# ViennaRNA/RNAcode

Measured on AMD Instinct MI355X. Metric: alignment-columns x samples scored /sec, higher is better.
Workload: dtype f32; 1 GPU; synthetic MAF 10000 blocks x 120 cols x 6 seqs, n=1000 (BASELINE configs[2]/[3]); exchange=none, fit_exp_mode=fused

## Files before the change

rnacode_amd/csrc/rc_batch.cpp:

```cpp
#include "rc_runtime.h"


extern "C" {

void rc_batch_destroy(rc_batch *b) {
  if (!b) return;
  trace("destroy", b);
  (void)hipSetDevice(b->device);
  const bool ctxAlive = b->ctx && !(b->retiredKeep && b->retiredKeep->ctxGone.load());
  if (b->state == rc_batch::RUNNING) { if (b->evDone.e) (void)hipEventSynchronize(b->evDone); if (ctxAlive) b->ctx->inflight.fetch_sub(1); }
  else if (b->state == rc_batch::READY && b->evPrep.e) (void)hipEventSynchronize(b->evPrep);
  delete b;
  trace("destroyed", b);
}

}


extern "C" void rc_batch_destroy(rc_batch *b);

int batch_prepare(rc_batch *b, const rc_block *blocks, int32_t n_blocks, const rc_params *par, const TableSet *set) {
  rc_ctx *ctx = b->ctx;
  if (par->blosum != 62 && par->blosum != 90) return fail(RC_ERR_ARG, "blosum must be 62 or 90");
  if (par->sampleN < 1) return fail(RC_ERR_ARG, "sampleN must be >= 1");
// ... 15 lines not shown
    if (blocks[i].n_rows >= 3 && blocks[i].n_rows <= kMaxRows && blocks[i].n_cols >= 3 && blocks[i].n_cols <= RC_MAX_COLS)
      block_footprint(blocks[i].n_rows, blocks[i].n_cols, &h, &d);
    hostSum += h; devSum += d;
  }
  const size_t nn = static_cast<size_t>(std::max(n_blocks, 1));
  const size_t tail = al256(nn * sizeof(DevBlock)) + 2 * al256(nn * sizeof(int)) + al256(nn * sizeof(uint64_t)) + al256((nn + 1) * sizeof(int));
  b->hostCap = al256(hostSum) + tail + 256;
  b->devCap = al256(devSum) + 256;
  HIP_TRY(hipSetDevice(ctx->device));
  HIP_TRY(b->hblob.ensure(b->hostCap));
  BlobArena arena;
  arena.host = b->hblob.as<uint8_t>();
  arena.hostCap = b->hostCap;
  arena.devCap = b->devCap;

  {
    if (!ctx->pool || ctx->pool->size() != ctx->hostThreads) ctx->pool.reset(new Pool(ctx->hostThreads));
    std::mutex errMu;
    ctx->pool->run(n_blocks, [&](int i) {
      std::string err;
      const int st = prepare_block(blocks[i], *par, pt, arena, static_cast<uint32_t>(i), b->db[i], b->meta[i], err);
      if (st != RC_OK && st != RC_ERR_SKIP) {
        std::lock_guard<std::mutex> lk(errMu);
        b->errs[i] = err;
      }
    });
  }

  bool sameL = true;
  const size_t SpadBytes = (static_cast<size_t>(par->sampleN) + kWave - 1) / kWave * kWave * sizeof(uint32_t);
  for (int i = 0; i < n_blocks; i++) {
    BlockMeta &m = b->meta[i];
    if (m.status != RC_OK) continue;
    if (static_cast<double>(b->db[i].nnodes) * m.cols * static_cast<double>(SpadBytes) > static_cast<double>(ctx->totalMem) / 4.0) {
      m.status = RC_ERR_UNSUPPORTED; b->db[i].status = RC_ERR_UNSUPPORTED;
      b->errs[i] = "rows x columns x samples too large for the device: the block's random-number streams (4 bytes x tree nodes x columns x samples) exceed a quarter of its memory; split the block (breakmaf) or lower --num-samples";
      continue;
    }
    b->okBlocks.push_back(i);
    auto &cls = b->classes[block_class(m.N, m.L, b->db[i].omega, ctx->rule)];
    if (!cls.empty() && b->meta[cls.front()].L != m.L) sameL = false;
    cls.push_back(i);
    b->maxL = std::max(b->maxL, m.L);
    b->maxDraws = std::max(b->maxDraws, b->db[i].nnodes * m.cols);
    const size_t smax = static_cast<size_t>(m.L) / 3;
    b->hssCap = std::max(b->hssCap, static_cast<int>(smax) / 3 + 2);
  }
  if (!sameL)
    for (auto &kv : b->classes) std::stable_sort(kv.second.begin(), kv.second.end(), [&](int x, int y) { return b->meta[x].L > b->meta[y].L; });
  for (auto &kv : b->classes)
    if (kv.first > kGenericClass) std::stable_sort(kv.second.begin(), kv.second.end(), [&](int x, int y) { return b->meta[x].NK > b->meta[y].NK; });

  uint8_t *base = arena.host;
  size_t o = al256(arena.hostUsed.load());
  auto take = [&](size_t bytes) { const size_t at = o; o += al256(bytes); return at; };
  b->oDblocks = take(nn * sizeof(DevBlock));
  b->oOk = take(nn * sizeof(int));
  b->oClass = take(nn * sizeof(int));
  b->oPrefix = take((nn + 1) * sizeof(int));
  if (o > b->hostCap) return fail(RC_ERR_ARG, "internal: blob tail does not fit");
  b->hostUsed = o;
  if (n_blocks > 0) std::memcpy(base + b->oDblocks, b->db.data(), sizeof(DevBlock) * n_blocks);
  if (!b->okBlocks.empty()) std::memcpy(base + b->oOk, b->okBlocks.data(), sizeof(int) * b->okBlocks.size());
  {
    int *cl = reinterpret_cast<int *>(base + b->oClass);
    int at = 0;
    std::fill(b->classOff, b->classOff + kClassSlots, 0);
// ... 337 lines not shown
```

rnacode_amd/csrc/rc_host.cpp:

```cpp
#include "rc_host.h"
#include "rc_refexp.h"

#include <algorithm>
#include <cmath>
#include <cstdlib>
#include <cstring>
#include <vector>

namespace rc {

static inline float f32(double x) { return static_cast<float>(x); }
static inline double f64(float x) { return static_cast<double>(x); }


namespace {
bool fast_decimal(const char *p, const char **end, double *out) {
  static const double pow10[23] = {1e0, 1e1, 1e2, 1e3, 1e4, 1e5, 1e6, 1e7, 1e8, 1e9, 1e10, 1e11, 1e12, 1e13, 1e14, 1e15, 1e16, 1e17, 1e18, 1e19, 1e20, 1e21, 1e22};
  const char *q = p;
  bool neg = false;
  if (*q == '-' || *q == '+') { neg = (*q == '-'); q++; }
  unsigned long long m = 0;
  int digits = 0, frac = 0, any = 0;
  for (; *q >= '0' && *q <= '9'; q++) { any = 1; if (m || *q != '0') { m = m * 10 + static_cast<unsigned>(*q - '0'); digits++; } if (digits > 15) return false; }
  if (*q == '.') {
    q++;
    for (; *q >= '0' && *q <= '9'; q++) { any = 1; m = m * 10 + static_cast<unsigned>(*q - '0'); if (m) digits++; frac++; if (digits > 15 || frac > 22) return false; }
  }
  if (!any || *q == 'e' || *q == 'E' || *q == 'x' || *q == 'X' || *q == 'p' || *q == 'P') return false;
  const double v = static_cast<double>(m) / pow10[frac];
  *out = neg ? -v : v;
  *end = q;
  return true;
}
// ... 410 lines not shown
    uint8_t *dst = chars + static_cast<size_t>(r) * cols;
    const uint8_t *src = reinterpret_cast<const uint8_t *>(in.rows[r]);
    for (int c = 0; c < cols; c++) dst[c] = luts.up[src[c]];
  }

  tip_distances(t, rowtip, N, dist, mark);
  float freqs[2][4];
  mono_freqs_both(chars, static_cast<size_t>(N) * cols, freqs[0], freqs[1]);
  ModelRec *models = reinterpret_cast<ModelRec *>(base + d.off_models);
  for (int s = 0; s < 2; s++)
    for (int j = 0; j < N; j++) {
      ModelRec &m = models[s * N + j];
      std::memset(&m, 0, sizeof m);
      m.dist = dist[j];
      m.kappa = in.kappa;
      std::memcpy(m.freqs, freqs[s], sizeof m.freqs);
      hky_probs(m.dist, m.freqs, m.kappa, m.P);
    }

  SeqGenHky hky(freqs[0], in.kappa);
  NodeRec *nodes = reinterpret_cast<NodeRec *>(base + d.off_nodes);
  for (int q = 0; q < t.nnodes; q++) {
    NodeRec &nr = nodes[q];
    std::memset(&nr, 0, sizeof nr);
    nr.parent = static_cast<uint16_t>(t.parent[q]);
    nr.gctrl = node_ctrl(static_cast<uint32_t>(t.parent[q])) | ((t.parent[q] >> 3) == (q >> 3) ? 0x80000000u : 0u);
    nr.tiprow = -1;
    double M[4][4];
    if (q != 0) hky.cumulative(t.length[q], M);
    for (int p = 0; p < 4; p++) {
      uint32_t b = 0;
      pack_thresholds(q == 0 ? hky.addFreq : M[p], &nr.thr[p], &b);
      nr.basepack |= b << (2 * p);
    }
  }
  uint8_t *qtip = base + d.off_qtip;
  uint16_t *qtip16 = reinterpret_cast<uint16_t *>(base + d.off_qtip16);
  std::memset(qtip, 0, sec.qtip);
  for (int r = 0; r < N; r++) {
    const int q = t.tipnode[rowtip[r]];
    qtip[r] = static_cast<uint8_t>(q);
    qtip16[r] = static_cast<uint16_t>(q);
    nodes[q].tiprow = static_cast<int16_t>(r);
  }
  return done(RC_OK);
}

int exp_mode_of_host() {
  bool fused = true, generic = true;
  uint64_t s = 88172645463325252ull;
  for (int i = 0; i < 20000 && (fused || generic); i++) {
    s ^= s << 13; s ^= s >> 7; s ^= s << 17;
    const double u = static_cast<double>(s >> 11) * (1.0 / 9007199254740992.0);
    const double x = (i & 3) == 3 ? 709.7 * u : -745.2 * u;
    const uint64_t want = exp_bits(std::exp(x));
    if (fused && exp_bits(ref_exp(x, true)) != want) fused = false;
    if (generic && exp_bits(ref_exp(x, false)) != want) generic = false;
  }
  return fused ? 2 : generic ? 1 : 0;
}

float pvalue_of(float score, float parMu, float parLambda) {
  const float arg = (-1) * parLambda * (score - parMu);
  return f32(1 - std::exp((-1) * std::exp(f64(arg))));
}

// ... 8 lines not shown
```

rnacode_amd/csrc/rc_null_generic.h:

```cpp
#pragma once
#include "rc_null_kernel.h"
#include "rc_null_tiled.h"

namespace rc {

struct GenericLayout {
  size_t offCodes;
  size_t offState;
  size_t offRow;
  size_t total;
  int nW;
  __host__ __device__ GenericLayout(int N, int L, int nn) {
    const size_t NK = static_cast<size_t>(N) - 1;
    nW = ((L / 3 + 31) >> 2) + 1;
    offCodes = 0;
    offState = (offCodes + 6 * NK * static_cast<size_t>(nW) * kWave * sizeof(uint32_t) + 255) & ~static_cast<size_t>(255);
    (void)nn;
    offRow = (offState + 2 * (3 * NK + 1) * kWave * sizeof(float) + 255) & ~static_cast<size_t>(255);
    total = (offRow + (static_cast<size_t>(L) / 3 + 8) * kWave * sizeof(float) + 255) & ~static_cast<size_t>(255);
  }
};

__host__ __device__ inline size_t generic_codes_bytes(int N, int L, int nn) { return GenericLayout(N, L, nn).offState; }
__host__ __device__ inline size_t generic_state_bytes(int N, int L, int nn) { const GenericLayout l(N, L, nn); return l.total - l.offState; }
// ... 157 lines not shown
#pragma unroll
          for (int t = 0; t < 8; t++) { u[t] = *up; up += qstride; }
        } else {
#pragma unroll
          for (int t = 0; t < 8; t++) {
            u[t] = 0u;
            if (q0 + t < nnodes) { u[t] = *up; up += qstride; }
          }
        }
        const int qa = q0 + thrNode < lastNode ? q0 + thrNode : lastNode, qb = q0 + 4 + thrNode < lastNode ? q0 + 4 + thrNode : lastNode;
        ta = nodew[qa * 20 + thrLane];
        tb = nodew[qb * 20 + thrLane];
        const int qc = q0 + (lane & 7) < lastNode ? q0 + (lane & 7) : lastNode;
        cv = nodew[qc * 20 + 16 + ((lane >> 3) & 3)];
      };
      fetch(0, uu, thrA, thrB, ctlV);
      for (int q0 = 0; q0 < nnodes; q0 += 8) {
        uint32_t un[8], tnA = 0u, tnB = 0u, cnV = 0u;
        if (q0 + 8 < nnodes) fetch(q0 + 8, un, tnA, tnB, cnV);
        const bool full = q0 + 8 <= nnodes;
        uint32_t cur = 0u;
        auto node = [&](auto tc) {
          constexpr int t = decltype(tc)::value;
          const uint32_t bp = static_cast<uint32_t>(__builtin_amdgcn_readlane(static_cast<int>(ctlV), t));
          const uint32_t ctl = static_cast<uint32_t>(__builtin_amdgcn_readlane(static_cast<int>(ctlV), 16 + t));
          uint32_t pw = cur;
          if (static_cast<int>(ctl) >= 0) pw = *reinterpret_cast<const uint16_t *>(ldsBytes + ((ctl & 0x7f80u) | laneSt));
          const uint32_t ps = (pw >> (ctl & 31u)) & 3u;
          const int at = static_cast<int>(ps << 4) + (t & 3) * 64;
          const int tv = static_cast<int>(t < 4 ? thrA : thrB);
          const uint32_t thx = static_cast<uint32_t>(__builtin_amdgcn_ds_bpermute(at, tv)), thy = static_cast<uint32_t>(__builtin_amdgcn_ds_bpermute(at + 4, tv)),
                         thz = static_cast<uint32_t>(__builtin_amdgcn_ds_bpermute(at + 8, tv)), thw = static_cast<uint32_t>(__builtin_amdgcn_ds_bpermute(at + 12, tv));
          const uint32_t u = uu[t];
          const uint32_t st = (u > thx) + (u > thy) + (u > thz) + ((bp >> (2 * ps)) & 3u);
          clamped += (u > thw);
          cur |= (st & 3u) << (2 * t);
        };
        if (full) {
          static_for<8>(node);
        } else {
          static_for<8>([&](auto tc) { if (q0 + decltype(tc)::value < nnodes) node(tc); });
        }
        *reinterpret_cast<uint16_t *>(ldsBytes + (static_cast<uint32_t>(q0 >> 3) * 128u + laneSt)) = static_cast<uint16_t>(cur);
#pragma unroll
        for (int t = 0; t < 8; t++) uu[t] = un[t];
        thrA = tnA; thrB = tnB; ctlV = cnV;
      }
      const int ip = L + 3 - i;
      const int jF = i / 3 - 1, jR = ip / 3 - 1;
      const uint32_t offF = (static_cast<uint32_t>(0 + i % 3) * NK * lay.nW + static_cast<uint32_t>(jF >> 2)) * (kWave * 4) + lane * 4 + (jF & 3);
      const uint32_t offR = (static_cast<uint32_t>(3 + ip % 3) * NK * lay.nW + static_cast<uint32_t>(jR >> 2)) * (kWave * 4) + lane * 4 + (jR & 3);
      const uint32_t *__restrict__ mrowF = maskw + static_cast<size_t>(0 * L1 + i) * NCW, *__restrict__ mrowR = maskw + static_cast<size_t>(1 * L1 + (i >= 3 ? ip : L)) * NCW;
      const bool emit = i >= 3;
      uint32_t aF, aR;
      {
        const uint32_t c = node_ctrl(qtip[0]);
        const uint32_t wv = *reinterpret_cast<const uint16_t *>(ldsBytes + ((c & 0x7f80u) | laneSt));
        aF = ((static_cast<uint32_t>(win[0]) << 2) | ((wv >> (c & 31u)) & 3u)) & 63u;
        win[0] = static_cast<uint8_t>(aF);
        aR = codon_flip(aF) ^ 63u;
      }
      const uint32_t aF64 = aF * 64u, aR64 = aR * 64u;
      uint8_t *__restrict__ kp = codes;
      const size_t kstep = static_cast<size_t>(lay.nW) * (kWave * 4);
      const int kChunk = TILED ? (kWave / A.tiledKT) * A.tiledKT : kWave;
      for (int k0 = 0; k0 < NK; k0 += kChunk) {
        const int kl = k0 + lane < NK ? k0 + lane : NK - 1;
        const uint32_t tctl = node_ctrl(qtip[kl + 1]);
        const uint32_t k5 = static_cast<uint32_t>(kl) / 5u, sh = 6u * (static_cast<uint32_t>(kl) - 5u * k5);
        const uint32_t mFv = (mrowF[k5] >> sh) & 63u, mRv = (mrowR[k5] >> sh) & 63u;
        const int nk = NK - k0 < kWave ? NK - k0 : kWave;
        if constexpr (TILED) {
          const TiledLayout tl(NK, A.tiledKT);
          uint32_t *__restrict__ cwp = reinterpret_cast<uint32_t *>(codes) + lane;
          const size_t posF = static_cast<size_t>(0 * L1 + i) * tl.WT * kWave, posR = static_cast<size_t>(1 * L1 + (emit ? ip : L)) * tl.WT * kWave;
          auto rowsT = [&](auto cnt, int kk, int widx) {
            constexpr int CNT = decltype(cnt)::value;
            uint32_t bb[CNT], cc[CNT], wv[CNT];
            uint8_t *wrow = win + (kk + 1) * kWave;
#pragma unroll
            for (int t = 0; t < CNT; t++) {
              cc[t] = static_cast<uint32_t>(__builtin_amdgcn_readlane(static_cast<int>(tctl), kk - k0 + t));
              wv[t] = *reinterpret_cast<const uint16_t *>(ldsBytes + ((cc[t] & 0x7f80u) | laneSt));
              bb[t] = wrow[t * kWave];
            }
#pragma unroll
            for (int t = 0; t < CNT; t++) bb[t] = ((bb[t] << 2) | ((wv[t] >> (cc[t] & 31u)) & 3u)) & 63u;
#pragma unroll
            for (int t = 0; t < CNT; t++) wrow[t * kWave] = static_cast<uint8_t>(bb[t]);
            if (emit) {
              uint32_t wf = 0u, wr = 0u;
#pragma unroll
              for (int t = 0; t < CNT; t++) {
                const uint32_t mF = static_cast<uint32_t>(__builtin_amdgcn_readlane(static_cast<int>(mFv), kk - k0 + t));
                const uint32_t mR = static_cast<uint32_t>(__builtin_amdgcn_readlane(static_cast<int>(mRv), kk - k0 + t));
                wf |= static_cast<uint32_t>(pairTab[aF64 + (bb[t] & mF)]) << (6 * t + 2);
                wr |= static_cast<uint32_t>(pairTab[aR64 + ((codon_flip(bb[t]) ^ 63u) & mR)]) << (6 * t + 2);
              }
              cwp[posF + static_cast<size_t>(widx) * kWave] = wf;
              cwp[posR + static_cast<size_t>(widx) * kWave] = wr;
            }
          };
          const int t0 = k0 / tl.KT, t1 = t0 + kChunk / tl.KT < tl.T ? t0 + kChunk / tl.KT : tl.T;
          for (int t = t0; t < t1; t++)
            for (int x = 0; x < tl.WPT; x++) {
              const int kk = t * tl.KT + 5 * x;
              int cnt = tl.KT - 5 * x;
              cnt = cnt > 5 ? 5 : cnt;
              cnt = cnt > NK - kk ? NK - kk : cnt;
              const int widx = t * tl.WPT + x;
              if (cnt >= 5) rowsT(std::integral_constant<int, 5>{}, kk, widx);
              else if (cnt == 4) rowsT(std::integral_constant<int, 4>{}, kk, widx);
              else if (cnt == 3) rowsT(std::integral_constant<int, 3>{}, kk, widx);
              else if (cnt == 2) rowsT(std::integral_constant<int, 2>{}, kk, widx);
              else if (cnt == 1) rowsT(std::integral_constant<int, 1>{}, kk, widx);
            }
          continue;
        }
        auto rows = [&](auto cnt, int kk) {
          constexpr int CNT = decltype(cnt)::value;
          uint32_t bb[CNT], pf[CNT], pr[CNT];
          uint8_t *wrow = win + (k0 + kk + 1) * kWave;
          uint32_t cc[CNT], wv[CNT];
#pragma unroll
          for (int t = 0; t < CNT; t++) {
            cc[t] = static_cast<uint32_t>(__builtin_amdgcn_readlane(static_cast<int>(tctl), kk + t));
            wv[t] = *reinterpret_cast<const uint16_t *>(ldsBytes + ((cc[t] & 0x7f80u) | laneSt));
            bb[t] = wrow[t * kWave];
          }
#pragma unroll
          for (int t = 0; t < CNT; t++) bb[t] = ((bb[t] << 2) | ((wv[t] >> (cc[t] & 31u)) & 3u)) & 63u;
#pragma unroll
          for (int t = 0; t < CNT; t++) wrow[t * kWave] = static_cast<uint8_t>(bb[t]);
          if (emit) {
#pragma unroll
            for (int t = 0; t < CNT; t++) {
              const uint32_t mF = static_cast<uint32_t>(__builtin_amdgcn_readlane(static_cast<int>(mFv), kk + t));
              const uint32_t mR = static_cast<uint32_t>(__builtin_amdgcn_readlane(static_cast<int>(mRv), kk + t));
              pf[t] = pairTab[aF64 + (bb[t] & mF)];
              pr[t] = pairTab[aR64 + ((codon_flip(bb[t]) ^ 63u) & mR)];
            }
#pragma unroll
            for (int t = 0; t < CNT; t++) {
              kp[offF] = static_cast<uint8_t>(pf[t] << 2);
              kp[offR] = static_cast<uint8_t>(pr[t] << 2);
              kp += kstep;
            }
          }
        };
        int kk = 0;
        for (; kk + 8 <= nk; kk += 8) rows(std::integral_constant<int, 8>{}, kk);
        for (; kk < nk; kk++) rows(std::integral_constant<int, 1>{}, kk);
      }
    }
    if (clamped && sidx < A.sampleN) atomicAdd(A.clampCount, static_cast<unsigned long long>(clamped));
    }
    if constexpr (SIM) continue;

    float best = -1.0f;
    const float negTie = -A.tieThr;
    const float *__restrict__ chainW = reinterpret_cast<const float *>(blob + db->off_chain);
    const uint32_t zeroCodes = (static_cast<uint32_t>(db->code_zero) << 2) * 0x01010101u;
    float *__restrict__ rowbuf = reinterpret_cast<float *>(mine + (lay.offRow - lay.offState)) + lane;
    float *__restrict__ dpB = dp + static_cast<size_t>(3 * NK + 1) * kWave;
    for (int s = 0; s < 2; s++)
      for (int f = 0; f < 3; f++) {
        const int sites = (L - f) / 3;
        if (sites <= 0) continue;
        if (onlyCombo >= 0 && onlyCombo != s * 3 + f) continue;
        SampleScan st{0.0f, 0.0f, 0u, 0u};
        for (int a = 0; a < sites; a += 2) {
          const int b = a + 1;
          sample_scan_row_begin(st, best, static_cast<uint32_t>(a));
          const int jendA = (a == sites - 1) ? sites - 1 : sites;
          const int jendB = (b >= sites - 1) ? sites - 1 : sites;
          uint32_t stickyA = nanSem ? 0xffffffffu : 0u, stickyB = stickyA;
          for (int j0 = a & ~3; j0 < jendA; j0 += kGenericTile) {
            const bool first = j0 <= a, more = j0 + kGenericTile < jendA;
// ... 173 lines not shown
```

rnacode_amd/csrc/rc_null_kernel.h:

```cpp
#pragma once
#include <hip/hip_runtime.h>

#include <type_traits>
#include <utility>

#include "rc_device.h"
#include "rc_launch.h"

namespace rc {


template <bool SEM> __device__ __forceinline__ float ref_max(float x, float y) {
  if constexpr (SEM) return x > y ? x : y;
  else return fmaxf(x, y);
}
template <bool SEM> __device__ __forceinline__ float ref_max3(float x, float y, float z) { return ref_max<SEM>(ref_max<SEM>(x, y), z); }

template <bool SEM = false>
__device__ __forceinline__ void pair_step(int zc, float sig, float Delta, float Omega, float omega,
                                          float &s0, float &s1, float &s2) {
  if (zc == 0) {
    s0 = s0 + sig;
    s1 = s1 + omega;
    s2 = s2 + omega;
  } else if (zc == 1) {
    const float n0 = ref_max<SEM>(s0 + Delta, s2 + Omega);
    const float n1 = ref_max<SEM>(s0 + Omega, s1 + Delta);
    const float n2 = ref_max<SEM>(s1 + Omega, s2 + Delta);
    s0 = n0; s1 = n1; s2 = n2;
  } else {
    const float n0 = ref_max<SEM>(s0 + Delta, s1 + Omega);
    const float n1 = ref_max<SEM>(s1 + Delta, s2 + Omega);
    const float n2 = ref_max<SEM>(s2 + Delta, s0 + Omega);
    s0 = n0; s1 = n1; s2 = n2;
  }
}

struct ScanState {
  float cm;
  int ss, se;
// ... 2 lines not shown
template <typename Emit>
__device__ __forceinline__ void scan_step(ScanState &st, float v, int a, int j, bool last, float tieThr, Emit emit) {
  if (v > 0.0f || last) {
    if ((st.cm > 0.0f && st.se < a) || last) {
      if (st.se - st.ss >= 2) emit(st);
      st.cm = v; st.ss = a; st.se = j;
    } else if (v > st.cm || (fabsf(v - st.cm) < tieThr && (j - a) >= (st.se - st.ss))) {
      st.cm = v; st.ss = a; st.se = j;
    }
  }
}

__device__ __forceinline__ void native_scan_rows(const float *rows, int aLo, int aHi, int sites, int s, int f, float tieThr, ScanState &st, int &n,
                                                 DevHss *out, int hssCap, int lane) {
  for (int a = aLo; a < aHi; a++) {
    for (int j0 = a; j0 < sites; j0 += kWave) {
      const int j = j0 + lane;
      const float v = (j < sites) ? rows[static_cast<size_t>(a - aLo) * sites + j] : 0.0f;
      const bool last = (a == sites - 1) && (j == sites - 1);
      unsigned long long m = __ballot((j < sites) && (v > 0.0f || last));
      while (m) {
        const int t = __builtin_ctzll(m);
        m &= m - 1ull;
        const int jj = j0 + t;
        const float vt = __int_as_float(__builtin_amdgcn_readlane(__float_as_int(v), t));
        scan_step(st, vt, a, jj, (a == sites - 1) && (jj == sites - 1), tieThr, [&](const ScanState &e) {
          if (out && lane == 0 && n < hssCap) out[n] = DevHss{s, f, e.ss, e.se, e.cm};
          n++;
        });
      }
    }
  }
}

__device__ __forceinline__ uint32_t codon_flip(uint32_t c) { return ((c & 3u) << 4) | (c & 12u) | ((c >> 4) & 3u); }


template <int K> struct KReg { float s0, s1, s2; int lut; };
template <typename Seq> struct KRegs;
template <int... K> struct KRegs<std::integer_sequence<int, K...>> : KReg<K>... {
  template <int I> __device__ __forceinline__ KReg<I> &at() { return static_cast<KReg<I> &>(*this); }
};
template <int NK, typename F, int... K>
__device__ __forceinline__ void static_for_impl(F &&f, std::integer_sequence<int, K...>) {
  (f(std::integral_constant<int, K>{}), ...);
}
template <int NK, typename F> __device__ __forceinline__ void static_for(F &&f) {
  static_for_impl<NK>(static_cast<F &&>(f), std::make_integer_sequence<int, NK>{});
}

template <int NK, bool EXACT> __device__ __forceinline__ float div_by_nk(float x, float nkf) {
  if constexpr ((NK & (NK - 1)) == 0) {
    return x * (1.0f / static_cast<float>(NK));
  } else if constexpr (EXACT) {
    return x / nkf;
  } else {
    constexpr float y = 1.0f / static_cast<float>(NK);
    const float q0 = x * y;
    const float r = __builtin_fmaf(-static_cast<float>(NK), q0, x);
    return __builtin_fmaf(r, y, q0);
  }
}

struct SampleScan {
  float cm;
  float Q;
  uint32_t se;
  uint32_t len;
// ... 149 lines not shown
    const float Delta = db->Delta, Omega = db->Omega, omega = db->omega, nkf = db->nkf;
    const NodeRec *__restrict__ nodes = reinterpret_cast<const NodeRec *>(blob + db->off_nodes);
    const uint32_t *__restrict__ qtipw = reinterpret_cast<const uint32_t *>(blob + db->off_qtip);
    const uint32_t *__restrict__ refcolw = reinterpret_cast<const uint32_t *>(blob + db->off_refcol);
    const unsigned long long *__restrict__ zw = reinterpret_cast<const unsigned long long *>(blob + db->off_zw);
    const unsigned long long *__restrict__ zmask = reinterpret_cast<const unsigned long long *>(blob + db->off_zmask);
    const int zmWords = db->zm_words;
    const uint32_t *__restrict__ maskw = reinterpret_cast<const uint32_t *>(blob + db->off_mask);
    const float *__restrict__ lut = reinterpret_cast<const float *>(blob + db->off_lut);
    const int sidx = grp * kWave + lane;
    const int L1 = L + 1;

    if (!ROWS && !helping && (!kProfiling || !(A.debugSkip & 2))) {
      constexpr int SPI = 4;
      constexpr int NODEW = (2 * N - 1 + 15) / 16;
      const U4 *thrTab;
      const uint8_t *pairLut;
      int thrStride;
      if constexpr (EXACT) {
        thrTab = reinterpret_cast<const U4 *>(nodes);
        thrStride = sizeof(NodeRec) / sizeof(U4);
        pairLut = pairTab;
      } else {
        thrTab = reinterpret_cast<const U4 *>(lds_codes);
        thrStride = 4;
        pairLut = reinterpret_cast<const uint8_t *>(lds_codes + nnodes * 16);
        const uint32_t *src = reinterpret_cast<const uint32_t *>(nodes);
        for (int idx = lane; idx < nnodes * 16; idx += kWave) lds_codes[idx] = src[(idx >> 4) * (sizeof(NodeRec) / 4) + (idx & 15)];
        const uint32_t *psrc = reinterpret_cast<const uint32_t *>(pairTab);
#pragma unroll
        for (int x = 0; x < 64 * 64 / 4 / kWave; x++) lds_codes[nnodes * 16 + x * kWave + lane] = psrc[x * kWave + lane];
      }
      const uint32_t *__restrict__ nodew = reinterpret_cast<const uint32_t *>(nodes);
      uint32_t win[N];
#pragma unroll
      for (int r = 0; r < N; r++) win[r] = 0;
      unsigned int clamped = 0;
      auto get_state = [&](const uint32_t (&ns)[NODEW], int q) -> uint32_t {
        uint32_t word = ns[0];
#pragma unroll
        for (int x = 1; x < NODEW; x++) if ((q >> 4) == x) word = ns[x];
        return (word >> (2 * (q & 15))) & 3u;
      };
      int iLo = 1, iHi = L;
      if constexpr (SIM) { iLo = 1 + static_cast<int>(static_cast<long long>(L) * rowPart / parts); iHi = static_cast<int>(static_cast<long long>(L) * (rowPart + 1) / parts); }
      for (int i0 = (SIM && iLo > 3) ? iLo - 2 : 1; i0 <= iHi; i0 += SPI) {
        size_t ubase[SPI];
        uint32_t ns[SPI][NODEW];
#pragma unroll
        for (int t = 0; t < SPI; t++) {
          const int i = (i0 + t <= L) ? i0 + t : L;
          const uint32_t col = (refcolw[i >> 1] >> (16 * (i & 1))) & 0xFFFFu;
          ubase[t] = static_cast<size_t>(col) * A.Spad + sidx;
#pragma unroll
          for (int x = 0; x < NODEW; x++) ns[t][x] = 0;
        }
        const size_t qstride = static_cast<size_t>(cols) * A.Spad;
        auto node_step = [&](int q, const uint32_t (&u)[SPI]) {
          const uint32_t bp = nodew[q * 20 + 16];
          const int pq = static_cast<int>(nodew[q * 20 + 17] & 255u);
          auto evolve = [&](auto withBase) {
#pragma unroll
            for (int t = 0; t < SPI; t++) {
              const uint32_t ps = (q == 0) ? 0u : get_state(ns[t], pq);
              const U4 th = thrTab[q * thrStride + ps];
              uint32_t st = (u[t] > th.x) + (u[t] > th.y) + (u[t] > th.z);
              if constexpr (decltype(withBase)::value) st += (bp >> (2 * ps)) & 3u;
              if constexpr (SIM) clamped += (u[t] > th.w) & (i0 + t >= iLo) & (i0 + t <= iHi); else clamped += (u[t] > th.w);
              const uint32_t bits = st << (2 * (q & 15));
#pragma unroll
              for (int x = 0; x < NODEW; x++) if (NODEW == 1 || (q >> 4) == x) ns[t][x] |= bits;
            }
          };
          if (__builtin_expect(bp != 0u, 0)) evolve(std::true_type{}); else evolve(std::false_type{});
        };
        if constexpr (SIM) {
          constexpr int QB = 8;
          for (int q0 = 0; q0 < nnodes; q0 += QB) {
            uint32_t ub[QB][SPI];
#pragma unroll
            for (int x = 0; x < QB; x++) {
              const int q = q0 + x < nnodes ? q0 + x : nnodes - 1;
#pragma unroll
              for (int t = 0; t < SPI; t++) ub[x][t] = Ustream[ubase[t] + q * qstride];
            }
#pragma unroll
            for (int x = 0; x < QB; x++) if (q0 + x < nnodes) node_step(q0 + x, ub[x]);
          }
        } else {
          for (int q = 0; q < nnodes; q++) {
            uint32_t u[SPI];
#pragma unroll
            for (int t = 0; t < SPI; t++) u[t] = Ustream[ubase[t] + q * qstride];
            node_step(q, u);
          }
        }
#pragma unroll
        for (int t = 0; t < SPI; t++) {
          const int i = i0 + t;
          if (i <= L) {
#pragma unroll
            for (int r = 0; r < N; r++) win[r] = (win[r] << 2) | get_state(ns[t], static_cast<int>((qtipw[r >> 2] >> (8 * (r & 3))) & 255u));
            if (i >= 3 && (!SIM || (i >= iLo && i <= iHi))) {
              const int ip = L + 3 - i;
              const uint32_t aF = win[0] & 63u;
              const uint32_t aR = codon_flip(aF) ^ 63u;
#pragma unroll
              for (int w = 0; w < NCW; w++) {
                uint32_t wf = 0, wr = 0;
                const uint32_t mF = maskw[(0 * L1 + i) * NCW + w], mR = maskw[(1 * L1 + ip) * NCW + w];
#pragma unroll
                for (int c = 0; c < CPW; c++) {
                  const int k = w * CPW + c;
                  if (k < NK) {
                    const uint32_t bF = win[k + 1] & ((mF >> (6 * c)) & 63u);
                    const uint32_t bR = (codon_flip(win[k + 1]) ^ 63u) & ((mR >> (6 * c)) & 63u);
                    wf |= static_cast<uint32_t>(pairLut[aF * 64 + bF]) << (6 * c + 2);
                    wr |= static_cast<uint32_t>(pairLut[aR * 64 + bR]) << (6 * c + 2);
                  }
                }
                if (w < NCW - 1) {
                  cod[static_cast<size_t>(0 * L1 + i) * PSW + w * kWave + lane] = wf;
                  cod[static_cast<size_t>(1 * L1 + ip) * PSW + w * kWave + lane] = wr;
                } else {
                  reinterpret_cast<TailT *>(cod + static_cast<size_t>(0 * L1 + i) * PSW + (NCW - 1) * kWave)[lane] = static_cast<TailT>(wf);
                  reinterpret_cast<TailT *>(cod + static_cast<size_t>(1 * L1 + ip) * PSW + (NCW - 1) * kWave)[lane] = static_cast<TailT>(wr);
                }
              }
            }
          }
        }
      }
      if (clamped && sidx < A.sampleN && (SIM || onlyCombo <= 0)) atomicAdd(A.clampCount, static_cast<unsigned long long>(clamped));
    }
    if constexpr (SIM) continue;
    if (!helping && shared) {
      const size_t G = gridDim.x;
      if (lane == 0) {
        __hip_atomic_store(A.steal + kStealHdr + G + 2 * blockIdx.x, static_cast<unsigned int>(bi), __ATOMIC_RELAXED, __HIP_MEMORY_SCOPE_AGENT);
        __hip_atomic_store(A.steal + kStealHdr + G + 2 * blockIdx.x + 1, static_cast<unsigned int>(grp), __ATOMIC_RELAXED, __HIP_MEMORY_SCOPE_AGENT);
      }
      __builtin_amdgcn_fence(__ATOMIC_RELEASE, "agent");
      __builtin_amdgcn_s_waitcnt(0);
      if (lane == 0) {
        atomicExch(A.steal + kStealHdr + blockIdx.x, 1u);
        const unsigned int idx = atomicAdd(A.steal, 1u);
        __hip_atomic_store(A.steal + kStealHdr + 3 * G + idx, (blockIdx.x + 1u) | (static_cast<unsigned int>(home) << 24), __ATOMIC_RELAXED, __HIP_MEMORY_SCOPE_AGENT);
        atomicSub(A.steal + 1, 1u);
      }
      firstCombo = claim_part(slot);
    }

    float best = -1.0f;
    unsigned long long statCells = 0, statNoPos = 0, statPosLanes = 0, statPristine = 0, statEvent = 0, statTail = 0;
    float omega_v, Delta_v = 0.0f;
    asm volatile("v_mov_b32 %0, %1" : "=v"(omega_v) : "s"(omega));
    float rcpNk_v = 0.0f, negNk_v = 0.0f;
    if constexpr (!EXACT && (NK & (NK - 1)) != 0) {
      asm volatile("v_mov_b32 %0, %1" : "=v"(rcpNk_v) : "s"(1.0f / static_cast<float>(NK)));
      asm volatile("v_mov_b32 %0, %1" : "=v"(negNk_v) : "s"(-static_cast<float>(NK)));
    }
    if constexpr (EXACT) asm volatile("v_mov_b32 %0, %1" : "=v"(Delta_v) : "s"(Delta));
    if (!kProfiling || !(A.debugSkip & 1)) {
      Regs R;
      int curS = -1;
      for (int c = onlyCombo >= 0 ? onlyCombo : firstCombo; c < 6; c = onlyCombo >= 0 ? 6 : (shared ? claim_part(slot) : c + 1)) {
// ... 761 lines not shown
```

Measured before the change: 28.20 billion alignment-columns*samples/s.

## Hand-schedule null-sim draw fetches, maintain reverse window, skip clamp counting when impossible

```diff
diff --git a/rnacode_amd/csrc/rc_batch.cpp b/rnacode_amd/csrc/rc_batch.cpp
--- a/rnacode_amd/csrc/rc_batch.cpp
+++ b/rnacode_amd/csrc/rc_batch.cpp
@@ -71,7 +71,7 @@
   for (int i = 0; i < n_blocks; i++) {
     BlockMeta &m = b->meta[i];
     if (m.status != RC_OK) continue;
-    if (static_cast<double>(b->db[i].nnodes) * m.cols * static_cast<double>(SpadBytes) > static_cast<double>(ctx->totalMem) / 4.0) {
+    if (static_cast<double>(b->db[i].nnodes) * m.cols * static_cast<double>(SpadBytes) > static_cast<double>(ctx->totalMem) / 4.0 || SpadBytes >= (1ull << 32)) {
       m.status = RC_ERR_UNSUPPORTED; b->db[i].status = RC_ERR_UNSUPPORTED;
       b->errs[i] = "rows x columns x samples too large for the device: the block's random-number streams (4 bytes x tree nodes x columns x samples) exceed a quarter of its memory; split the block (breakmaf) or lower --num-samples";
       continue;
diff --git a/rnacode_amd/csrc/rc_host.cpp b/rnacode_amd/csrc/rc_host.cpp
--- a/rnacode_amd/csrc/rc_host.cpp
+++ b/rnacode_amd/csrc/rc_host.cpp
@@ -1,4 +1,5 @@
 #include "rc_host.h"
+#include "rc_sim_core.h"
 #include "rc_refexp.h"
 
 #include <algorithm>
@@ -475,6 +476,7 @@
       uint32_t b = 0;
       pack_thresholds(q == 0 ? hky.addFreq : M[p], &nr.thr[p], &b);
       nr.basepack |= b << (2 * p);
+      if (sim_may_clamp(nr.thr[p].w)) nr.parent |= kNodeMayClamp;
     }
   }
   uint8_t *qtip = base + d.off_qtip;
diff --git a/rnacode_amd/csrc/rc_null_generic.h b/rnacode_amd/csrc/rc_null_generic.h
--- a/rnacode_amd/csrc/rc_null_generic.h
+++ b/rnacode_amd/csrc/rc_null_generic.h
@@ -213,8 +213,8 @@
           const uint32_t thx = static_cast<uint32_t>(__builtin_amdgcn_ds_bpermute(at, tv)), thy = static_cast<uint32_t>(__builtin_amdgcn_ds_bpermute(at + 4, tv)),
                          thz = static_cast<uint32_t>(__builtin_amdgcn_ds_bpermute(at + 8, tv)), thw = static_cast<uint32_t>(__builtin_amdgcn_ds_bpermute(at + 12, tv));
           const uint32_t u = uu[t];
-          const uint32_t st = (u > thx) + (u > thy) + (u > thz) + ((bp >> (2 * ps)) & 3u);
-          clamped += (u > thw);
+          const uint32_t st = sim_draw(u, thx, thy, thz) + sim_base(bp, ps);
+          clamped += sim_clamps(u, thw);
           cur |= (st & 3u) << (2 * t);
         };
         if (full) {
@@ -237,11 +237,10 @@
       {
         const uint32_t c = node_ctrl(qtip[0]);
         const uint32_t wv = *reinterpret_cast<const uint16_t *>(ldsBytes + ((c & 0x7f80u) | laneSt));
-        aF = ((static_cast<uint32_t>(win[0]) << 2) | ((wv >> (c & 31u)) & 3u)) & 63u;
+        aF = sim_window6(win[0], (wv >> (c & 31u)) & 3u);
         win[0] = static_cast<uint8_t>(aF);
-        aR = codon_flip(aF) ^ 63u;
+        aR = sim_ref_rev(aF);
       }
-      const uint32_t aF64 = aF * 64u, aR64 = aR * 64u;
       uint8_t *__restrict__ kp = codes;
       const size_t kstep = static_cast<size_t>(lay.nW) * (kWave * 4);
       const int kChunk = TILED ? (kWave / A.tiledKT) * A.tiledKT : kWave;
@@ -266,7 +265,7 @@
               bb[t] = wrow[t * kWave];
             }
 #pragma unroll
-            for (int t = 0; t < CNT; t++) bb[t] = ((bb[t] << 2) | ((wv[t] >> (cc[t] & 31u)) & 3u)) & 63u;
+            for (int t = 0; t < CNT; t++) bb[t] = sim_window6(bb[t], (wv[t] >> (cc[t] & 31u)) & 3u);
 #pragma unroll
             for (int t = 0; t < CNT; t++) wrow[t * kWave] = static_cast<uint8_t>(bb[t]);
             if (emit) {
@@ -275,8 +274,8 @@
               for (int t = 0; t < CNT; t++) {
                 const uint32_t mF = static_cast<uint32_t>(__builtin_amdgcn_readlane(static_cast<int>(mFv), kk - k0 + t));
                 const uint32_t mR = static_cast<uint32_t>(__builtin_amdgcn_readlane(static_cast<int>(mRv), kk - k0 + t));
-                wf |= static_cast<uint32_t>(pairTab[aF64 + (bb[t] & mF)]) << (6 * t + 2);
-                wr |= static_cast<uint32_t>(pairTab[aR64 + ((codon_flip(bb[t]) ^ 63u) & mR)]) << (6 * t + 2);
+                wf |= sim_pack(pairTab[sim_index_fwd(aF, bb[t], mF)], t);
+                wr |= sim_pack(pairTab[sim_index_rev(aR, bb[t], mR)], t);
               }
               cwp[posF + static_cast<size_t>(widx) * kWave] = wf;
               cwp[posR + static_cast<size_t>(widx) * kWave] = wr;
@@ -310,7 +309,7 @@
             bb[t] = wrow[t * kWave];
           }
 #pragma unroll
-          for (int t = 0; t < CNT; t++) bb[t] = ((bb[t] << 2) | ((wv[t] >> (cc[t] & 31u)) & 3u)) & 63u;
+          for (int t = 0; t < CNT; t++) bb[t] = sim_window6(bb[t], (wv[t] >> (cc[t] & 31u)) & 3u);
 #pragma unroll
           for (int t = 0; t < CNT; t++) wrow[t * kWave] = static_cast<uint8_t>(bb[t]);
           if (emit) {
@@ -318,13 +317,13 @@
             for (int t = 0; t < CNT; t++) {
               const uint32_t mF = static_cast<uint32_t>(__builtin_amdgcn_readlane(static_cast<int>(mFv), kk + t));
               const uint32_t mR = static_cast<uint32_t>(__builtin_amdgcn_readlane(static_cast<int>(mRv), kk + t));
-              pf[t] = pairTab[aF64 + (bb[t] & mF)];
-              pr[t] = pairTab[aR64 + ((codon_flip(bb[t]) ^ 63u) & mR)];
+              pf[t] = pairTab[sim_index_fwd(aF, bb[t], mF)];
+              pr[t] = pairTab[sim_index_rev(aR, bb[t], mR)];
             }
 #pragma unroll
             for (int t = 0; t < CNT; t++) {
-              kp[offF] = static_cast<uint8_t>(pf[t] << 2);
-              kp[offR] = static_cast<uint8_t>(pr[t] << 2);
+              kp[offF] = static_cast<uint8_t>(sim_pack(pf[t], 0));
+              kp[offR] = static_cast<uint8_t>(sim_pack(pr[t], 0));
               kp += kstep;
             }
           }
diff --git a/rnacode_amd/csrc/rc_null_kernel.h b/rnacode_amd/csrc/rc_null_kernel.h
--- a/rnacode_amd/csrc/rc_null_kernel.h
+++ b/rnacode_amd/csrc/rc_null_kernel.h
@@ -6,6 +6,7 @@
 
 #include "rc_device.h"
 #include "rc_launch.h"
+#include "rc_sim_core.h"
 
 namespace rc {
 
@@ -74,8 +75,6 @@
     }
   }
 }
-
-__device__ __forceinline__ uint32_t codon_flip(uint32_t c) { return ((c & 3u) << 4) | (c & 12u) | ((c >> 4) & 3u); }
 
 
 template <int K> struct KReg { float s0, s1, s2; int lut; };
@@ -291,10 +290,45 @@
         for (int x = 0; x < 64 * 64 / 4 / kWave; x++) lds_codes[nnodes * 16 + x * kWave + lane] = psrc[x * kWave + lane];
       }
       const uint32_t *__restrict__ nodew = reinterpret_cast<const uint32_t *>(nodes);
-      uint32_t win[N];
+      constexpr bool kRevWindow = N <= 16;
+      constexpr bool kLean = N <= 16;
+      uint32_t win[N], winR[kRevWindow ? N : 1];
 #pragma unroll
       for (int r = 0; r < N; r++) win[r] = 0;
+#pragma unroll
+      for (int r = 0; r < (kRevWindow ? N : 1); r++) winR[r] = 0;
       unsigned int clamped = 0;
+      const uint32_t laneDraw = static_cast<uint32_t>(sidx) * 4u;
+      const uint32_t laneWord = static_cast<uint32_t>(lane) * 4u, laneTailB = static_cast<uint32_t>(lane) * LB;
+      auto fetch_draws = [&](uint32_t (&u)[4], const uint8_t *b0, const uint8_t *b1, const uint8_t *b2, const uint8_t *b3) {
+#ifdef RC_PLAIN_FETCH
+        u[0] = *reinterpret_cast<const uint32_t *>(b0 + laneDraw); u[1] = *reinterpret_cast<const uint32_t *>(b1 + laneDraw);
+        u[2] = *reinterpret_cast<const uint32_t *>(b2 + laneDraw); u[3] = *reinterpret_cast<const uint32_t *>(b3 + laneDraw);
+#else
+        asm volatile("s_nop 4\n\tglobal_load_dword %0, %4, %5\n\tglobal_load_dword %1, %4, %6\n\tglobal_load_dword %2, %4, %7\n\tglobal_load_dword %3, %4, %8"
+                     : "=&v"(u[0]), "=&v"(u[1]), "=&v"(u[2]), "=&v"(u[3]) : "v"(laneDraw), "s"(b0), "s"(b1), "s"(b2), "s"(b3));
+#endif
+      };
+      auto wait_draws = [&](uint32_t (&u)[4], auto younger) {
+#ifndef RC_PLAIN_FETCH
+        asm volatile("s_waitcnt vmcnt(%4)" : "+v"(u[0]), "+v"(u[1]), "+v"(u[2]), "+v"(u[3]) : "n"(decltype(younger)::value));
+#endif
+      };
+      auto store_words = [&](auto tail, uint32_t off, uint32_t wf, uint32_t wr, uint8_t *bF, uint8_t *bR) {
+        constexpr int W = decltype(tail)::value;
+#ifdef RC_PLAIN_FETCH
+        constexpr bool kPlain = true;
+#else
+        constexpr bool kPlain = !kLean;
+#endif
+        if constexpr (kPlain) {
+          using T = std::conditional_t<W == 1, uint8_t, std::conditional_t<W == 2, uint16_t, uint32_t>>;
+          *reinterpret_cast<T *>(bF + off) = static_cast<T>(wf);
+          *reinterpret_cast<T *>(bR + off) = static_cast<T>(wr);
+        } else if constexpr (W == 1) asm volatile("s_nop 4\n\tglobal_store_byte %0, %1, %3\n\tglobal_store_byte %0, %2, %4" : : "v"(off), "v"(wf), "v"(wr), "s"(bF), "s"(bR) : "memory");
+        else if constexpr (W == 2) asm volatile("s_nop 4\n\tglobal_store_short %0, %1, %3\n\tglobal_store_short %0, %2, %4" : : "v"(off), "v"(wf), "v"(wr), "s"(bF), "s"(bR) : "memory");
+        else asm volatile("s_nop 4\n\tglobal_store_dword %0, %1, %3\n\tglobal_store_dword %0, %2, %4" : : "v"(off), "v"(wf), "v"(wr), "s"(bF), "s"(bR) : "memory");
+      };
       auto get_state = [&](const uint32_t (&ns)[NODEW], int q) -> uint32_t {
         uint32_t word = ns[0];
 #pragma unroll
@@ -304,18 +338,21 @@
       int iLo = 1, iHi = L;
       if constexpr (SIM) { iLo = 1 + static_cast<int>(static_cast<long long>(L) * rowPart / parts); iHi = static_cast<int>(static_cast<long long>(L) * (rowPart + 1) / parts); }
       for (int i0 = (SIM && iLo > 3) ? iLo - 2 : 1; i0 <= iHi; i0 += SPI) {
+        static_assert(SPI == 4, "fetch_draws / wait_draws: four sites per pass");
+        const uint8_t *ub[SPI];
         size_t ubase[SPI];
         uint32_t ns[SPI][NODEW];
 #pragma unroll
         for (int t = 0; t < SPI; t++) {
           const int i = (i0 + t <= L) ? i0 + t : L;
           const uint32_t col = (refcolw[i >> 1] >> (16 * (i & 1))) & 0xFFFFu;
+          ub[t] = reinterpret_cast<const uint8_t *>(Ustream + static_cast<size_t>(col) * A.Spad);
           ubase[t] = static_cast<size_t>(col) * A.Spad + sidx;
 #pragma unroll
           for (int x = 0; x < NODEW; x++) ns[t][x] = 0;
         }
-        const size_t qstride = static_cast<size_t>(cols) * A.Spad;
-        auto node_step = [&](int q, const uint32_t (&u)[SPI]) {
+        const size_t qstride = static_cast<size_t>(cols) * A.Spad, qstrideB = qstride * sizeof(uint32_t);
+        auto node_step_plain = [&](int q, const uint32_t (&u)[SPI]) {
           const uint32_t bp = nodew[q * 20 + 16];
           const int pq = static_cast<int>(nodew[q * 20 + 17] & 255u);
           auto evolve = [&](auto withBase) {
@@ -323,35 +360,111 @@
             for (int t = 0; t < SPI; t++) {
               const uint32_t ps = (q == 0) ? 0u : get_state(ns[t], pq);
               const U4 th = thrTab[q * thrStride + ps];
-              uint32_t st = (u[t] > th.x) + (u[t] > th.y) + (u[t] > th.z);
-              if constexpr (decltype(withBase)::value) st += (bp >> (2 * ps)) & 3u;
-              if constexpr (SIM) clamped += (u[t] > th.w) & (i0 + t >= iLo) & (i0 + t <= iHi); else clamped += (u[t] > th.w);
+              uint32_t st = sim_draw(u[t], th.x, th.y, th.z);
+              if constexpr (decltype(withBase)::value) st += sim_base(bp, ps);
+              if constexpr (SIM) clamped += sim_clamps(u[t], th.w) & (i0 + t >= iLo) & (i0 + t <= iHi); else clamped += sim_clamps(u[t], th.w);
               const uint32_t bits = st << (2 * (q & 15));
 #pragma unroll
               for (int x = 0; x < NODEW; x++) if (NODEW == 1 || (q >> 4) == x) ns[t][x] |= bits;
             }
           };
           if (__builtin_expect(bp != 0u, 0)) evolve(std::true_type{}); else evolve(std::false_type{});
+        };
+        auto node_step = [&](int q, uint32_t (&u)[SPI], auto &&arrived) {
+          const uint32_t bp = nodew[q * 20 + 16];
+          const uint32_t w17 = nodew[q * 20 + 17];
+          const int pq = static_cast<int>(w17 & 255u);
+          {
+            uint32_t ps[SPI], st[SPI];
+            U4 th[SPI];
+#pragma unroll
+            for (int t = 0; t < SPI; t++) {
+              ps[t] = (q == 0) ? 0u : get_state(ns[t], pq);
+              th[t] = thrTab[q * thrStride + ps[t]];
+            }
+            arrived();
+#ifndef RC_PLAIN_FETCH
+            {
+              unsigned long long m0, m1, m2, m3;
+              asm("v_cmp_gt_u32_e64 %4, %8, %12\n\tv_cmp_gt_u32_e64 %5, %9, %15\n\tv_cmp_gt_u32_e64 %6, %10, %18\n\tv_cmp_gt_u32_e64 %7, %11, %21\n\t"
+                  "v_cndmask_b32_e64 %0, 0, 1, %4\n\tv_cndmask_b32_e64 %1, 0, 1, %5\n\tv_cndmask_b32_e64 %2, 0, 1, %6\n\tv_cndmask_b32_e64 %3, 0, 1, %7\n\t"
+                  "v_cmp_gt_u32_e64 %4, %8, %13\n\tv_cmp_gt_u32_e64 %5, %9, %16\n\tv_cmp_gt_u32_e64 %6, %10, %19\n\tv_cmp_gt_u32_e64 %7, %11, %22\n\t"
+                  "v_addc_co_u32_e64 %0, %4, 0, %0, %4\n\tv_addc_co_u32_e64 %1, %5, 0, %1, %5\n\tv_addc_co_u32_e64 %2, %6, 0, %2, %6\n\tv_addc_co_u32_e64 %3, %7, 0, %3, %7\n\t"
+                  "v_cmp_gt_u32_e64 %4, %8, %14\n\tv_cmp_gt_u32_e64 %5, %9, %17\n\tv_cmp_gt_u32_e64 %6, %10, %20\n\tv_cmp_gt_u32_e64 %7, %11, %23\n\t"
+                  "v_addc_co_u32_e64 %0, %4, 0, %0, %4\n\tv_addc_co_u32_e64 %1, %5, 0, %1, %5\n\tv_addc_co_u32_e64 %2, %6, 0, %2, %6\n\tv_addc_co_u32_e64 %3, %7, 0, %3, %7"
+                  : "=&v"(st[0]), "=&v"(st[1]), "=&v"(st[2]), "=&v"(st[3]), "=&s"(m0), "=&s"(m1), "=&s"(m2), "=&s"(m3)
+                  : "v"(u[0]), "v"(u[1]), "v"(u[2]), "v"(u[3]), "v"(th[0].x), "v"(th[0].y), "v"(th[0].z), "v"(th[1].x), "v"(th[1].y), "v"(th[1].z),
+                    "v"(th[2].x), "v"(th[2].y), "v"(th[2].z), "v"(th[3].x), "v"(th[3].y), "v"(th[3].z));
+            }
+#else
+#pragma unroll
+            for (int t = 0; t < SPI; t++) st[t] = sim_draw(u[t], th[t].x, th[t].y, th[t].z);
+#endif
+            if (w17 & kNodeMayClamp) {
+              auto clamp_mask = [&](int t) -> unsigned long long {
+                const unsigned long long m = __ballot(sim_clamps(u[t], th[t].w) != 0u);
+                if constexpr (SIM) return (i0 + t >= iLo && i0 + t <= iHi) ? m : 0ull; else return m;
+              };
+              unsigned long long any = 0;
+#pragma unroll
+              for (int t = 0; t < SPI; t++) any |= clamp_mask(t);
+              if (__builtin_expect(any != 0ull, 0)) {
+                const unsigned long long live = __ballot(sidx < A.sampleN);
+#pragma unroll
+                for (int t = 0; t < SPI; t++) clamped += static_cast<unsigned int>(__builtin_popcountll(clamp_mask(t) & live));
+              }
+            }
+            if (__builtin_expect(bp != 0u, 0)) {
+#pragma unroll
+              for (int t = 0; t < SPI; t++) st[t] += sim_base(bp, ps[t]);
+            }
+#pragma unroll
+            for (int t = 0; t < SPI; t++) {
+              const uint32_t bits = st[t] << (2 * (q & 15));
+#pragma unroll
+              for (int x = 0; x < NODEW; x++) if (NODEW == 1 || (q >> 4) == x) ns[t][x] |= bits;
+            }
+          }
         };
         if constexpr (SIM) {
           constexpr int QB = 8;
           for (int q0 = 0; q0 < nnodes; q0 += QB) {
-            uint32_t ub[QB][SPI];
+            uint32_t ubq[QB][SPI];
+            if constexpr (!kLean) {
+#pragma unroll
+              for (int x = 0; x < QB; x++) {
+                const int q = q0 + x < nnodes ? q0 + x : nnodes - 1;
+#pragma unroll
+                for (int t = 0; t < SPI; t++) ubq[x][t] = Ustream[ubase[t] + q * qstride];
+              }
+#pragma unroll
+              for (int x = 0; x < QB; x++) if (q0 + x < nnodes) node_step_plain(q0 + x, ubq[x]);
+              continue;
+            }
 #pragma unroll
             for (int x = 0; x < QB; x++) {
-              const int q = q0 + x < nnodes ? q0 + x : nnodes - 1;
-#pragma unroll
-              for (int t = 0; t < SPI; t++) ub[x][t] = Ustream[ubase[t] + q * qstride];
-            }
-#pragma unroll
-            for (int x = 0; x < QB; x++) if (q0 + x < nnodes) node_step(q0 + x, ub[x]);
+              const size_t at = static_cast<size_t>(q0 + x < nnodes ? q0 + x : nnodes - 1) * qstrideB;
+              fetch_draws(ubq[x], ub[0] + at, ub[1] + at, ub[2] + at, ub[3] + at);
+            }
+            static_for<QB>([&](auto xc) {
+              constexpr int x = decltype(xc)::value;
+              wait_draws(ubq[x], std::integral_constant<int, SPI * (QB - 1 - x)>{});
+              if (q0 + x < nnodes) node_step(q0 + x, ubq[x], [] {});
+            });
           }
         } else {
           for (int q = 0; q < nnodes; q++) {
             uint32_t u[SPI];
-#pragma unroll
-            for (int t = 0; t < SPI; t++) u[t] = Ustream[ubase[t] + q * qstride];
-            node_step(q, u);
+            if constexpr (!kLean) {
+#pragma unroll
+              for (int t = 0; t < SPI; t++) u[t] = Ustream[ubase[t] + q * qstride];
+              node_step_plain(q, u);
+              continue;
+            }
+            fetch_draws(u, ub[0], ub[1], ub[2], ub[3]);
+#pragma unroll
+            for (int t = 0; t < SPI; t++) ub[t] += qstrideB;
+            node_step(q, u, [&] { wait_draws(u, std::integral_constant<int, 0>{}); });
           }
         }
 #pragma unroll
@@ -359,11 +472,18 @@
           const int i = i0 + t;
           if (i <= L) {
 #pragma unroll
-            for (int r = 0; r < N; r++) win[r] = (win[r] << 2) | get_state(ns[t], static_cast<int>((qtipw[r >> 2] >> (8 * (r & 3))) & 255u));
+            for (int r = 0; r < N; r++) {
+              const uint32_t tip = get_state(ns[t], static_cast<int>((qtipw[r >> 2] >> (8 * (r & 3))) & 255u));
+              win[r] = sim_window(win[r], tip);
+              if constexpr (kRevWindow) winR[r] = sim_window_rev(winR[r], tip);
+            }
             if (i >= 3 && (!SIM || (i >= iLo && i <= iHi))) {
               const int ip = L + 3 - i;
               const uint32_t aF = win[0] & 63u;
-              const uint32_t aR = codon_flip(aF) ^ 63u;
+              uint32_t aR = kRevWindow ? sim_rev_codon(winR[0]) : sim_ref_rev(aF);
+              asm("" : "+v"(aR));
+              uint8_t *siteF = reinterpret_cast<uint8_t *>(cod + static_cast<size_t>(0 * L1 + i) * PSW);
+              uint8_t *siteR = reinterpret_cast<uint8_t *>(cod + static_cast<size_t>(1 * L1 + ip) * PSW);
 #pragma unroll
               for (int w = 0; w < NCW; w++) {
                 uint32_t wf = 0, wr = 0;
@@ -372,25 +492,22 @@
                 for (int c = 0; c < CPW; c++) {
                   const int k = w * CPW + c;
                   if (k < NK) {
-                    const uint32_t bF = win[k + 1] & ((mF >> (6 * c)) & 63u);
-                    const uint32_t bR = (codon_flip(win[k + 1]) ^ 63u) & ((mR >> (6 * c)) & 63u);
-                    wf |= static_cast<uint32_t>(pairLut[aF * 64 + bF]) << (6 * c + 2);
-                    wr |= static_cast<uint32_t>(pairLut[aR * 64 + bR]) << (6 * c + 2);
+                    wf |= sim_pack(pairLut[sim_index_fwd(aF, win[k + 1], sim_mask_field(mF, c))], c);
+                    if constexpr (kRevWindow) wr |= sim_pack(pairLut[sim_index_rev_window(aR, winR[k + 1], sim_mask_field(mR, c))], c);
+                    else wr |= sim_pack(pairLut[sim_index_rev(aR, win[k + 1], sim_mask_field(mR, c))], c);
                   }
                 }
                 if (w < NCW - 1) {
-                  cod[static_cast<size_t>(0 * L1 + i) * PSW + w * kWave + lane] = wf;
-                  cod[static_cast<size_t>(1 * L1 + ip) * PSW + w * kWave + lane] = wr;
+                  store_words(std::integral_constant<int, 4>{}, laneWord, wf, wr, siteF + w * kWave * 4, siteR + w * kWave * 4);
                 } else {
-                  reinterpret_cast<TailT *>(cod + static_cast<size_t>(0 * L1 + i) * PSW + (NCW - 1) * kWave)[lane] = static_cast<TailT>(wf);
-                  reinterpret_cast<TailT *>(cod + static_cast<size_t>(1 * L1 + ip) * PSW + (NCW - 1) * kWave)[lane] = static_cast<TailT>(wr);
+                  store_words(std::integral_constant<int, LB>{}, laneTailB, wf, wr, siteF + (NCW - 1) * kWave * 4, siteR + (NCW - 1) * kWave * 4);
                 }
               }
             }
           }
         }
       }
-      if (clamped && sidx < A.sampleN && (SIM || onlyCombo <= 0)) atomicAdd(A.clampCount, static_cast<unsigned long long>(clamped));
+      if (clamped && (kLean ? lane == 0 : sidx < A.sampleN) && (SIM || onlyCombo <= 0)) atomicAdd(A.clampCount, static_cast<unsigned long long>(clamped));
     }
     if constexpr (SIM) continue;
     if (!helping && shared) {
diff --git a/rnacode_amd/csrc/rc_sim_core.h b/rnacode_amd/csrc/rc_sim_core.h
--- /dev/null
+++ b/rnacode_amd/csrc/rc_sim_core.h
@@ -0,0 +1,33 @@
+#pragma once
+#include <cstdint>
+
+#ifdef __HIPCC__
+#define RC_SIM_HD __host__ __device__ __forceinline__
+#else
+#define RC_SIM_HD inline
+#endif
+
+namespace rc {
+
+RC_SIM_HD uint32_t codon_flip(uint32_t c) { return ((c & 3u) << 4) | (c & 12u) | ((c >> 4) & 3u); }
+
+RC_SIM_HD uint32_t sim_draw(uint32_t u, uint32_t t0, uint32_t t1, uint32_t t2) { return (u > t0) + (u > t1) + (u > t2); }
+RC_SIM_HD uint32_t sim_base(uint32_t basepack, uint32_t ps) { return (basepack >> (2 * ps)) & 3u; }
+RC_SIM_HD uint32_t sim_clamps(uint32_t u, uint32_t t3) { return u > t3; }
+constexpr uint32_t kNodeMayClamp = 0x8000u;
+RC_SIM_HD bool sim_may_clamp(uint32_t t3) { return t3 != 0xFFFFFFFFu; }
+
+RC_SIM_HD uint32_t sim_window(uint32_t win, uint32_t state) { return (win << 2) | state; }
+RC_SIM_HD uint32_t sim_window6(uint32_t win, uint32_t state) { return ((win << 2) | state) & 63u; }
+
+RC_SIM_HD uint32_t sim_window_rev(uint32_t winR, uint32_t state) { return (state << 4) | (winR >> 2); }
+RC_SIM_HD uint32_t sim_rev_codon(uint32_t winR) { return winR ^ 63u; }
+
+RC_SIM_HD uint32_t sim_ref_rev(uint32_t aF) { return codon_flip(aF) ^ 63u; }
+RC_SIM_HD uint32_t sim_index_fwd(uint32_t aF, uint32_t b, uint32_t m) { return aF * 64u + (b & m); }
+RC_SIM_HD uint32_t sim_index_rev(uint32_t aR, uint32_t b, uint32_t m) { return aR * 64u + ((codon_flip(b) ^ 63u) & m); }
+RC_SIM_HD uint32_t sim_index_rev_window(uint32_t aR, uint32_t winR, uint32_t m) { return aR * 64u + ((winR ^ 63u) & m); }
+RC_SIM_HD uint32_t sim_mask_field(uint32_t word, int c) { return (word >> (6 * c)) & 63u; }
+RC_SIM_HD uint32_t sim_pack(uint32_t code, int c) { return code << (6 * c + 2); }
+
+}
```

Result: faster. 28.65 billion alignment-columns*samples/s (median of 6 runs) (+1.6%).
